# StarRocks/starrocks

Hardware: AMD Instinct MI355X
Metric: ssb_join_agg_rows_per_sec (higher is better)
Workload: dtype int64; 1 GPU; ssb_sf100_q21_star_groupby; rows_per_gpu=600000000, seed=42, parallelism=dp1-replicated-dims

## Files before the change

starrocks_amd/csrc/gpue.hip:

```cpp
#include <hip/hip_runtime.h>
#include <cstdio>
#include <cstring>
#include <cstdlib>
#include <thread>
#include "gpue.h"

static thread_local char g_err[512] = {0};

const char* gpue_last_error(void) { return g_err; }

#define HIP_CHECK(expr)                                                      \
    do {                                                                     \
        hipError_t _e = (expr);                                              \
        if (_e != hipSuccess) {                                              \
            snprintf(g_err, sizeof(g_err), "%s failed: %s (%s:%d)", #expr,   \
                     hipGetErrorString(_e), __FILE__, __LINE__);             \
            return GPUE_ERR_HIP;                                             \
        }                                                                    \
    } while (0)

#define ARG_CHECK(cond)                                                      \
    do {                                                                     \
        if (!(cond)) {                                                       \
            snprintf(g_err, sizeof(g_err), "bad argument: %s (%s:%d)",       \
// ... 3907 lines not shown
    uint32_t wqn = 0;
    const uint64_t n4 = n / 4;
    const int4* __restrict__ pk4 = (const int4*)pk;
    const int4* __restrict__ sk4 = (const int4*)sk;
    const int4* __restrict__ od4 = (const int4*)od;
    const int4* __restrict__ rv4 = (const int4*)rv;
    uint64_t stride = (uint64_t)gridDim.x * blockDim.x;
    auto ld4 = [&](const int4* p, uint64_t i) {
        const uint64_t* q = (const uint64_t*)(p + i);
        uint64_t lo = __builtin_nontemporal_load(q);
        uint64_t hi = __builtin_nontemporal_load(q + 1);
        int4 v;
        v.x = (int32_t)lo; v.y = (int32_t)(lo >> 32);
        v.z = (int32_t)hi; v.w = (int32_t)(hi >> 32);
        return v;
    };
    auto drain64 = [&]() {
        int4 e = wq[wid][wqn - 64 + lane];
        uint32_t brand1 = pfirst[e.x - 1];
        if (brand1) {
            uint32_t sidx = (uint32_t)(e.y - ssmin);
            if (sidx < ssint && ((sbits[sidx >> 5] >> (sidx & 31)) & 1u)) {
                uint32_t year1 = dfirst[e.z - dmin];
                atomicAdd(&g[(year1 - 1) * 1000 + (brand1 - 1)],
                          (unsigned long long)(int64_t)e.w);
            }
        }
        wqn -= 64;
    };
    auto quad = [&](int4 p4, int4 s4, int4 o4, int4 r4, bool inb) {
        #pragma unroll
        for (int j = 0; j < 4; j++) {
            uint32_t idx = (uint32_t)((&p4.x)[j] - psmin);
            bool in = inb & (idx < psint);
            uint32_t fidx = (in ? idx : 0u) & PF_MASK;
            bool maybe = in & (pf[fidx >> 5] >> (fidx & 31)) & 1u;
            uint64_t m = __ballot(maybe);
            if (m) {
                uint32_t rank = __popcll(m & ((1ull << lane) - 1));
                if (maybe)
                    wq[wid][wqn + rank] =
                        make_int4((&p4.x)[j], (&s4.x)[j], (&o4.x)[j], (&r4.x)[j]);
                wqn += __popcll(m);
                if (wqn >= 64) drain64();
            }
        }
    };
    uint64_t base = (uint64_t)blockIdx.x * blockDim.x + (uint64_t)wid * WAVE;
    uint64_t i = base + lane;
    for (; base + stride + WAVE <= n4; base += 2 * stride, i += 2 * stride) {
        int4 pa = ld4(pk4, i), sa = ld4(sk4, i), oa = ld4(od4, i), ra = ld4(rv4, i);
        uint64_t i2 = i + stride;
        int4 pb_ = ld4(pk4, i2), sb = ld4(sk4, i2), ob = ld4(od4, i2), rb = ld4(rv4, i2);
        quad(pa, sa, oa, ra, true);
        quad(pb_, sb, ob, rb, true);
    }
    for (; base < n4; base += stride, i += stride) {
        bool inb = i < n4;
        int4 z = make_int4(0, 0, 0, 0);
        int4 p4 = inb ? pk4[i] : z, s4 = inb ? sk4[i] : z;
        int4 o4 = inb ? od4[i] : z, r4 = inb ? rv4[i] : z;
        quad(p4, s4, o4, r4, inb);
    }
    if (wqn > 0 && lane < (int)wqn) {
        int4 e = wq[wid][lane];
        uint32_t brand1 = pfirst[e.x - 1];
        if (brand1) {
            uint32_t sidx = (uint32_t)(e.y - ssmin);
            if (sidx < ssint && ((sbits[sidx >> 5] >> (sidx & 31)) & 1u)) {
                uint32_t year1 = dfirst[e.z - dmin];
                atomicAdd(&g[(year1 - 1) * 1000 + (brand1 - 1)],
                          (unsigned long long)(int64_t)e.w);
            }
        }
    }
    uint64_t tid = (uint64_t)blockIdx.x * blockDim.x + threadIdx.x;
    for (uint64_t r = n4 * 4 + tid; r < n; r += stride) {
        uint32_t idx = (uint32_t)(pk[r] - psmin);
        if (idx >= psint) continue;
        uint32_t fidx = idx & PF_MASK;
        if (!((pf[fidx >> 5] >> (fidx & 31)) & 1u)) continue;
        uint32_t brand1 = pfirst[pk[r] - 1];
        if (!brand1) continue;
        uint32_t sidx = (uint32_t)(sk[r] - ssmin);
        if (sidx >= ssint || !((sbits[sidx >> 5] >> (sidx & 31)) & 1u)) continue;
        uint32_t year1 = dfirst[od[r] - dmin];
        atomicAdd(&g[(year1 - 1) * 1000 + (brand1 - 1)], (unsigned long long)(int64_t)rv[r]);
    }
    __syncthreads();
    for (int j = threadIdx.x; j < NG_Q21; j += blockDim.x)
        if (g[j] != 0) atomicAdd(&group_sums[j], g[j]);
}

__global__ __launch_bounds__(BLOCK_Q21) void
k_q21_star_agg_pfq2(const int32_t* __restrict__ pk, const int32_t* __restrict__ sk,
                   const int32_t* __restrict__ od, const int32_t* __restrict__ rv,
                   uint64_t n, const uint32_t* __restrict__ prefilter, int64_t psmin,
                   uint64_t psint, const uint16_t* __restrict__ pfirst,
                   const uint32_t* __restrict__ sbits, int64_t ssmin, uint64_t ssint,
                   const uint16_t* __restrict__ dfirst, int64_t dmin,
                   unsigned long long* __restrict__ group_sums) {
    __shared__ uint32_t pfa[1 << 13];
    __shared__ uint32_t pfb[1 << 13];
    __shared__ unsigned long long g[NG_Q21];
    __shared__ int4 wq[BLOCK_Q21 / WAVE][128];
    for (uint32_t w = threadIdx.x; w < (1u << 13); w += blockDim.x) {
        pfa[w] = prefilter[w];
        pfb[w] = prefilter[(1u << 13) + w];
    }
    for (int j = threadIdx.x; j < NG_Q21; j += blockDim.x) g[j] = 0;
    __syncthreads();
    const int wid = threadIdx.x / WAVE;
    const int lane = threadIdx.x & (WAVE - 1);
    uint32_t wqn = 0;
    const uint64_t n4 = n / 4;
    const int4* __restrict__ pk4 = (const int4*)pk;
    const int4* __restrict__ sk4 = (const int4*)sk;
    const int4* __restrict__ od4 = (const int4*)od;
    const int4* __restrict__ rv4 = (const int4*)rv;
    uint64_t stride = (uint64_t)gridDim.x * blockDim.x;
    auto ld4 = [&](const int4* p, uint64_t i) {
        const uint64_t* q = (const uint64_t*)(p + i);
        uint64_t lo = __builtin_nontemporal_load(q);
        uint64_t hi = __builtin_nontemporal_load(q + 1);
        int4 v;
        v.x = (int32_t)lo; v.y = (int32_t)(lo >> 32);
        v.z = (int32_t)hi; v.w = (int32_t)(hi >> 32);
        return v;
    };
    auto drain64 = [&]() {
        int4 e = wq[wid][wqn - 64 + lane];
        uint32_t brand1 = pfirst[e.x - 1];
        if (brand1) {
            uint32_t sidx = (uint32_t)(e.y - ssmin);
            if (sidx < ssint && ((sbits[sidx >> 5] >> (sidx & 31)) & 1u)) {
                uint32_t year1 = dfirst[e.z - dmin];
                atomicAdd(&g[(year1 - 1) * 1000 + (brand1 - 1)],
                          (unsigned long long)(int64_t)e.w);
            }
        }
        wqn -= 64;
    };
    auto quad = [&](int4 p4, int4 s4, int4 o4, int4 r4, bool inb) {
        #pragma unroll
        for (int j = 0; j < 4; j++) {
            uint32_t idx = (uint32_t)((&p4.x)[j] - psmin);
            bool in = inb & (idx < psint);
            uint32_t ia = (in ? idx : 0u) & ((1u << 18) - 1);
            uint32_t ib = ((in ? idx : 0u) * 2654435761u) >> 14;
            bool maybe = in & (pfa[ia >> 5] >> (ia & 31)) & (pfb[ib >> 5] >> (ib & 31)) & 1u;
            uint64_t m = __ballot(maybe);
            if (m) {
                uint32_t rank = __popcll(m & ((1ull << lane) - 1));
                if (maybe)
                    wq[wid][wqn + rank] =
                        make_int4((&p4.x)[j], (&s4.x)[j], (&o4.x)[j], (&r4.x)[j]);
                wqn += __popcll(m);
                if (wqn >= 64) drain64();
            }
        }
    };
    uint64_t base = (uint64_t)blockIdx.x * blockDim.x + (uint64_t)wid * WAVE;
    uint64_t i = base + lane;
    for (; base + stride + WAVE <= n4; base += 2 * stride, i += 2 * stride) {
        int4 pa = ld4(pk4, i), sa = ld4(sk4, i), oa = ld4(od4, i), ra = ld4(rv4, i);
        uint64_t i2 = i + stride;
        int4 pb_ = ld4(pk4, i2), sb = ld4(sk4, i2), ob = ld4(od4, i2), rb = ld4(rv4, i2);
        quad(pa, sa, oa, ra, true);
        quad(pb_, sb, ob, rb, true);
    }
    for (; base < n4; base += stride, i += stride) {
        bool inb = i < n4;
        int4 z = make_int4(0, 0, 0, 0);
        int4 p4 = inb ? pk4[i] : z, s4 = inb ? sk4[i] : z;
        int4 o4 = inb ? od4[i] : z, r4 = inb ? rv4[i] : z;
        quad(p4, s4, o4, r4, inb);
    }
    if (wqn > 0 && lane < (int)wqn) {
        int4 e = wq[wid][lane];
        uint32_t brand1 = pfirst[e.x - 1];
        if (brand1) {
            uint32_t sidx = (uint32_t)(e.y - ssmin);
            if (sidx < ssint && ((sbits[sidx >> 5] >> (sidx & 31)) & 1u)) {
                uint32_t year1 = dfirst[e.z - dmin];
                atomicAdd(&g[(year1 - 1) * 1000 + (brand1 - 1)],
                          (unsigned long long)(int64_t)e.w);
            }
        }
    }
    uint64_t tid = (uint64_t)blockIdx.x * blockDim.x + threadIdx.x;
    for (uint64_t r = n4 * 4 + tid; r < n; r += stride) {
        uint32_t idx = (uint32_t)(pk[r] - psmin);
        if (idx >= psint) continue;
        uint32_t ia = idx & ((1u << 18) - 1);
        uint32_t ib = (idx * 2654435761u) >> 14;
        if (!((pfa[ia >> 5] >> (ia & 31)) & (pfb[ib >> 5] >> (ib & 31)) & 1u)) continue;
        uint32_t brand1 = pfirst[pk[r] - 1];
        if (!brand1) continue;
        uint32_t sidx = (uint32_t)(sk[r] - ssmin);
        if (sidx >= ssint || !((sbits[sidx >> 5] >> (sidx & 31)) & 1u)) continue;
        uint32_t year1 = dfirst[od[r] - dmin];
        atomicAdd(&g[(year1 - 1) * 1000 + (brand1 - 1)], (unsigned long long)(int64_t)rv[r]);
    }
    __syncthreads();
    for (int j = threadIdx.x; j < NG_Q21; j += blockDim.x)
        if (g[j] != 0) atomicAdd(&group_sums[j], g[j]);
}


__global__ __launch_bounds__(BLOCK_Q21) void
k_q21_star_agg_pfq3(const int32_t* __restrict__ pk, const int32_t* __restrict__ sk,
                    const int32_t* __restrict__ od, const int32_t* __restrict__ rv,
                    uint64_t n, const uint32_t* __restrict__ prefilter, int64_t psmin,
                    uint64_t psint, const uint16_t* __restrict__ pfirst,
                    const uint32_t* __restrict__ sbits, int64_t ssmin, uint64_t ssint,
                    const uint16_t* __restrict__ dfirst, int64_t dmin,
                    unsigned long long* __restrict__ group_sums) {
    __shared__ uint32_t pfa[1 << 13];
    __shared__ uint32_t pfb[1 << 13];
    __shared__ unsigned long long g[NG_Q21];
    __shared__ int2 wq[BLOCK_Q21 / WAVE][128];
    for (uint32_t w = threadIdx.x; w < (1u << 13); w += blockDim.x) {
        pfa[w] = prefilter[w];
        pfb[w] = prefilter[(1u << 13) + w];
    }
    for (int j = threadIdx.x; j < NG_Q21; j += blockDim.x) g[j] = 0;
    __syncthreads();
    const int wid = threadIdx.x / WAVE;
    const int lane = threadIdx.x & (WAVE - 1);
    uint32_t wqn = 0;
    const uint64_t n4 = n / 4;
    const int4* __restrict__ pk4 = (const int4*)pk;
    uint64_t stride = (uint64_t)gridDim.x * blockDim.x;
    auto process = [&](int2 e) {
        uint32_t brand1 = pfirst[e.x - 1];
        if (!brand1) return;
        uint32_t r = (uint32_t)e.y;
        uint32_t sidx = (uint32_t)(sk[r] - ssmin);
        if (sidx >= ssint || !((sbits[sidx >> 5] >> (sidx & 31)) & 1u)) return;
        uint32_t year1 = dfirst[od[r] - dmin];
        atomicAdd(&g[(year1 - 1) * 1000 + (brand1 - 1)],
                  (unsigned long long)(int64_t)rv[r]);
    };
    auto push = [&](int32_t key, uint32_t row, bool inb) {
        uint32_t idx = (uint32_t)(key - psmin);
        bool in = inb & (idx < psint);
        uint32_t ia = (in ? idx : 0u) & ((1u << 18) - 1);
        uint32_t ib = ((in ? idx : 0u) * 2654435761u) >> 14;
        bool maybe = in & (pfa[ia >> 5] >> (ia & 31)) & (pfb[ib >> 5] >> (ib & 31)) & 1u;
        uint64_t m = __ballot(maybe);
        if (m) {
            uint32_t rank = __popcll(m & ((1ull << lane) - 1));
            if (maybe) wq[wid][wqn + rank] = make_int2(key, (int32_t)row);
            wqn += __popcll(m);
            if (wqn >= 64) {
                process(wq[wid][wqn - 64 + lane]);
                wqn -= 64;
            }
        }
    };
    auto ld4nt = [&](const int4* p, uint64_t i) {
        const uint64_t* q = (const uint64_t*)(p + i);
        uint64_t lo = __builtin_nontemporal_load(q);
        uint64_t hi = __builtin_nontemporal_load(q + 1);
        int4 v;
        v.x = (int32_t)lo; v.y = (int32_t)(lo >> 32);
        v.z = (int32_t)hi; v.w = (int32_t)(hi >> 32);
        return v;
    };
    uint64_t base = (uint64_t)blockIdx.x * blockDim.x + (uint64_t)wid * WAVE;
    uint64_t i = base + lane;
    for (; base + stride + WAVE <= n4; base += 2 * stride, i += 2 * stride) {
        int4 pa = ld4nt(pk4, i);
        uint64_t i2 = i + stride;
        int4 pb_ = ld4nt(pk4, i2);
        #pragma unroll
        for (int j = 0; j < 4; j++) push((&pa.x)[j], (uint32_t)(i * 4 + j), true);
        #pragma unroll
        for (int j = 0; j < 4; j++) push((&pb_.x)[j], (uint32_t)(i2 * 4 + j), true);
    }
    for (; base < n4; base += stride, i += stride) {
        bool inb = i < n4;
        int4 p4 = inb ? pk4[i] : make_int4(0, 0, 0, 0);
        #pragma unroll
        for (int j = 0; j < 4; j++) push((&p4.x)[j], (uint32_t)(i * 4 + j), inb);
    }
    if (wqn > 0 && lane < (int)wqn) process(wq[wid][lane]);
    uint64_t tid = (uint64_t)blockIdx.x * blockDim.x + threadIdx.x;
    for (uint64_t r = n4 * 4 + tid; r < n; r += stride) {
        uint32_t idx = (uint32_t)(pk[r] - psmin);
        if (idx >= psint) continue;
        uint32_t brand1 = pfirst[pk[r] - 1];
        if (!brand1) continue;
        uint32_t sidx = (uint32_t)(sk[r] - ssmin);
        if (sidx >= ssint || !((sbits[sidx >> 5] >> (sidx & 31)) & 1u)) continue;
        uint32_t year1 = dfirst[od[r] - dmin];
        atomicAdd(&g[(year1 - 1) * 1000 + (brand1 - 1)], (unsigned long long)(int64_t)rv[r]);
    }
    __syncthreads();
    for (int j = threadIdx.x; j < NG_Q21; j += blockDim.x)
        if (g[j] != 0) atomicAdd(&group_sums[j], g[j]);
}

__global__ void k_q21_pass_payload(const int32_t* __restrict__ pk, uint64_t n,
                                   const uint32_t* __restrict__ pbits, int64_t psmin,
                                   uint64_t psint, const uint16_t* __restrict__ pfirst,
                                   uint16_t* __restrict__ brand_out) {
    const uint64_t n4 = n / 4;
    const int4* __restrict__ pk4 = (const int4*)pk;
    uint64_t stride = (uint64_t)gridDim.x * blockDim.x;
    uint64_t i = (uint64_t)blockIdx.x * blockDim.x + threadIdx.x;
    for (; i + stride < n4; i += 2 * stride) {
        int4 pa = pk4[i];
        int4 pb_ = pk4[i + stride];
        ushort4 oa, ob;
        #pragma unroll
        for (int j = 0; j < 4; j++) {
            uint32_t idx = (uint32_t)((&pa.x)[j] - psmin);
            bool in = idx < psint;
            uint32_t cidx = in ? idx : 0u;
            bool pass = in & ((pbits[cidx >> 5] >> (cidx & 31)) & 1u);
            (&oa.x)[j] = pass ? pfirst[(&pa.x)[j] - 1] : (uint16_t)0;
        }
        #pragma unroll
        for (int j = 0; j < 4; j++) {
            uint32_t idx = (uint32_t)((&pb_.x)[j] - psmin);
            bool in = idx < psint;
            uint32_t cidx = in ? idx : 0u;
            bool pass = in & ((pbits[cidx >> 5] >> (cidx & 31)) & 1u);
            (&ob.x)[j] = pass ? pfirst[(&pb_.x)[j] - 1] : (uint16_t)0;
        }
        ((ushort4*)brand_out)[i] = oa;
        ((ushort4*)brand_out)[i + stride] = ob;
    }
    for (; i < n4; i += stride) {
        int4 p4 = pk4[i];
        ushort4 o;
        #pragma unroll
        for (int j = 0; j < 4; j++) {
            uint32_t idx = (uint32_t)((&p4.x)[j] - psmin);
            bool in = idx < psint;
            uint32_t cidx = in ? idx : 0u;
            bool pass = in & ((pbits[cidx >> 5] >> (cidx & 31)) & 1u);
            (&o.x)[j] = pass ? pfirst[(&p4.x)[j] - 1] : (uint16_t)0;
        }
        ((ushort4*)brand_out)[i] = o;
    }
    uint64_t tid = (uint64_t)blockIdx.x * blockDim.x + threadIdx.x;
    for (uint64_t r = n4 * 4 + tid; r < n; r += stride) {
        uint32_t idx = (uint32_t)(pk[r] - psmin);
        bool in = idx < psint;
        uint32_t cidx = in ? idx : 0u;
        bool pass = in & ((pbits[cidx >> 5] >> (cidx & 31)) & 1u);
        brand_out[r] = pass ? pfirst[pk[r] - 1] : (uint16_t)0;
    }
}

__global__ __launch_bounds__(BLOCK_Q21) void
k_q21_phase2(const uint16_t* __restrict__ brand, const int32_t* __restrict__ sk,
             const int32_t* __restrict__ od, const int32_t* __restrict__ rv, uint64_t n,
             const uint32_t* __restrict__ sbits, int64_t ssmin, uint64_t ssint,
             const uint16_t* __restrict__ dfirst, int64_t dmin,
             unsigned long long* __restrict__ group_sums) {
    __shared__ unsigned long long g[NG_Q21];
    for (int j = threadIdx.x; j < NG_Q21; j += blockDim.x) g[j] = 0;
    __syncthreads();
    const uint64_t n4 = n / 4;
    const ushort4* __restrict__ br4 = (const ushort4*)brand;
    const int4* __restrict__ sk4 = (const int4*)sk;
    const int4* __restrict__ od4 = (const int4*)od;
    const int4* __restrict__ rv4 = (const int4*)rv;
    uint64_t stride = (uint64_t)gridDim.x * blockDim.x;
    for (uint64_t i = (uint64_t)blockIdx.x * blockDim.x + threadIdx.x; i < n4; i += stride) {
        ushort4 b4 = br4[i];
        int4 s4 = sk4[i];
        int4 o4 = od4[i];
        int4 r4 = rv4[i];
        #pragma unroll
        for (int j = 0; j < 4; j++) {
            uint16_t brand1 = (&b4.x)[j];
            if (brand1 == 0) continue;
            uint32_t sidx = (uint32_t)((&s4.x)[j] - ssmin);
            if (sidx >= ssint || !((sbits[sidx >> 5] >> (sidx & 31)) & 1u)) continue;
            uint32_t year1 = dfirst[(&o4.x)[j] - dmin];
            atomicAdd(&g[(year1 - 1) * 1000 + (brand1 - 1)],
                      (unsigned long long)(int64_t)(&r4.x)[j]);
        }
    }
    uint64_t tid = (uint64_t)blockIdx.x * blockDim.x + threadIdx.x;
    for (uint64_t r = n4 * 4 + tid; r < n; r += stride) {
        uint16_t brand1 = brand[r];
        if (brand1 == 0) continue;
        uint32_t sidx = (uint32_t)(sk[r] - ssmin);
        if (sidx >= ssint || !((sbits[sidx >> 5] >> (sidx & 31)) & 1u)) continue;
        uint32_t year1 = dfirst[od[r] - dmin];
        atomicAdd(&g[(year1 - 1) * 1000 + (brand1 - 1)], (unsigned long long)(int64_t)rv[r]);
    }
    __syncthreads();
    for (int j = threadIdx.x; j < NG_Q21; j += blockDim.x)
        if (g[j] != 0) atomicAdd(&group_sums[j], g[j]);
}

extern "C" int gpue_q21_star_agg_pipe(gpue_session* s, gpue_join_table* parts,
                                      gpue_join_table* supps, gpue_join_table* dates,
                                      gpue_dbuf* pk, gpue_dbuf* sk, gpue_dbuf* od,
                                      gpue_dbuf* rv, uint64_t n, gpue_dbuf* brand_scratch,
                                      gpue_dbuf* group_sums, int n_chunks);
int gpue_q21_star_agg_pipe(gpue_session* s, gpue_join_table* parts, gpue_join_table* supps,
                           gpue_join_table* dates, gpue_dbuf* pk, gpue_dbuf* sk,
                           gpue_dbuf* od, gpue_dbuf* rv, uint64_t n,
                           gpue_dbuf* brand_scratch, gpue_dbuf* group_sums, int n_chunks) {
    ARG_CHECK(s && parts && supps && dates && pk && sk && od && rv && brand_scratch &&
              group_sums);
    ARG_CHECK(parts->first16 && parts->bitset && supps->bitset && dates->first16);
    ARG_CHECK(brand_scratch->bytes >= n * 2);
    ARG_CHECK(n_chunks >= 1 && n_chunks <= gpue_session::N_CHUNK_EVENTS);
    HIP_CHECK(hipMemsetAsync(group_sums->ptr, 0, NG_Q21 * sizeof(int64_t), s->stream));
    uint64_t per = (n + (uint64_t)n_chunks - 1) / (uint64_t)n_chunks;
    uint64_t chunk = (per + 3) & ~3ull;
    for (int c = 0; c < n_chunks; c++) {
        uint64_t lo = (uint64_t)c * chunk;
        if (lo >= n) break;
        uint64_t len = min(chunk, n - lo);
        hipLaunchKernelGGL(k_q21_pass_payload, dim3(grid_for(len)), dim3(BLOCK), 0,
                           s->stream2, (const int32_t*)pk->ptr + lo, len, parts->bitset,
                           parts->set_min, (uint64_t)(parts->set_max - parts->set_min + 1),
                           parts->first16, (uint16_t*)brand_scratch->ptr + lo);
        HIP_CHECK(hipEventRecord(s->chunk_ev[c], s->stream2));
        HIP_CHECK(hipStreamWaitEvent(s->stream, s->chunk_ev[c], 0));
        hipLaunchKernelGGL(k_q21_phase2, dim3(env_cap("GPUE_GRID_WIDE", 512)),
                           dim3(BLOCK_Q21), 0, s->stream,
                           (const uint16_t*)brand_scratch->ptr + lo,
                           (const int32_t*)sk->ptr + lo, (const int32_t*)od->ptr + lo,
                           (const int32_t*)rv->ptr + lo, len, supps->bitset,
                           supps->set_min, (uint64_t)(supps->set_max - supps->set_min + 1),
                           dates->first16, dates->min_key,
                           (unsigned long long*)group_sums->ptr);
    }
    HIP_CHECK(hipGetLastError());
    return GPUE_OK;
}

static bool q21_glob() {
    static int v = -1;
    if (v < 0) {
        const char* e = getenv("GPUE_Q21_GLOB");
        v = (e && atoi(e)) ? 1 : 0;
    }
    return v == 1;
}

static bool q21_pf() {
    static int v = -1;
    if (v < 0) {
        const char* e = getenv("GPUE_Q21_PF");
        v = (e && !atoi(e)) ? 0 : 1;
    }
    return v == 1;
}

extern "C" int gpue_q21_star_agg_async(gpue_session* s, gpue_join_table* parts,
                                       gpue_join_table* supps, gpue_join_table* dates,
                                       gpue_dbuf* pk, gpue_dbuf* sk, gpue_dbuf* od,
                                       gpue_dbuf* rv, uint64_t n, gpue_dbuf* group_sums);
int gpue_q21_star_agg_async(gpue_session* s, gpue_join_table* parts, gpue_join_table* supps,
                            gpue_join_table* dates, gpue_dbuf* pk, gpue_dbuf* sk,
                            gpue_dbuf* od, gpue_dbuf* rv, uint64_t n, gpue_dbuf* group_sums) {
    ARG_CHECK(s && parts && supps && dates && pk && sk && od && rv && group_sums);
    ARG_CHECK(group_sums->bytes >= NG_Q21 * sizeof(int64_t));
    ARG_CHECK(parts->min_key == 1 && supps->min_key == 1);
    ARG_CHECK(parts->first16 && supps->first16 && dates->first16);
    HIP_CHECK(hipMemsetAsync(group_sums->ptr, 0, NG_Q21 * sizeof(int64_t), s->stream));
    if (q21_pf() && parts->prefilter) {
        const char* e = getenv("GPUE_Q21_PF");
        int mode = e ? atoi(e) : 7;
        const char* nt = getenv("GPUE_Q21_PF_NT");
        bool use_nt = !nt || atoi(nt);
        int def_grid = mode == 2 ? 512 : 256;
        int tpb = env_cap("GPUE_Q21_PF_TPB", BLOCK_Q21);
        auto launch = [&](auto kern, int grid) {
            hipLaunchKernelGGL(kern, dim3(env_cap("GPUE_GRID_PF", grid)),
                               dim3(tpb), 0, s->stream, (const int32_t*)pk->ptr,
                               (const int32_t*)sk->ptr, (const int32_t*)od->ptr,
                               (const int32_t*)rv->ptr, n, parts->prefilter, parts->set_min,
                               (uint64_t)(parts->set_max - parts->set_min + 1),
                               parts->first16, supps->bitset, supps->set_min,
                               (uint64_t)(supps->set_max - supps->set_min + 1),
                               dates->first16, dates->min_key,
                               (unsigned long long*)group_sums->ptr);
        };
        if (mode == 7) {
            hipLaunchKernelGGL(k_q21_star_agg_pfq3, dim3(env_cap("GPUE_GRID_PF", def_grid)),
                               dim3(tpb), 0, s->stream, (const int32_t*)pk->ptr,
                               (const int32_t*)sk->ptr, (const int32_t*)od->ptr,
                               (const int32_t*)rv->ptr, n, parts->prefilter2,
                               parts->set_min,
                               (uint64_t)(parts->set_max - parts->set_min + 1),
                               parts->first16, supps->bitset, supps->set_min,
                               (uint64_t)(supps->set_max - supps->set_min + 1),
                               dates->first16, dates->min_key,
                               (unsigned long long*)group_sums->ptr);
        }
        else if (mode == 6) {
            hipLaunchKernelGGL(k_q21_star_agg_pfq2, dim3(env_cap("GPUE_GRID_PF", def_grid)),
                               dim3(tpb), 0, s->stream, (const int32_t*)pk->ptr,
                               (const int32_t*)sk->ptr, (const int32_t*)od->ptr,
                               (const int32_t*)rv->ptr, n, parts->prefilter2,
                               parts->set_min,
                               (uint64_t)(parts->set_max - parts->set_min + 1),
                               parts->first16, supps->bitset, supps->set_min,
                               (uint64_t)(supps->set_max - supps->set_min + 1),
                               dates->first16, dates->min_key,
                               (unsigned long long*)group_sums->ptr);
        }
        else if (mode == 4) launch(k_q21_star_agg_pfq, def_grid);
        else if (mode == 2 && use_nt) launch(k_q21_star_agg_pf<false, true>, def_grid);
        else if (mode == 2) launch(k_q21_star_agg_pf<false, false>, def_grid);
        else if (use_nt) launch(k_q21_star_agg_pf<true, true>, def_grid);
        else launch(k_q21_star_agg_pf<true, false>, def_grid);
        HIP_CHECK(hipGetLastError());
        return GPUE_OK;
    }
    if (q21_glob()) {
        hipLaunchKernelGGL(k_q21_star_agg_glob, dim3(grid_stream(n)), dim3(BLOCK), 0,
                           s->stream, (const int32_t*)pk->ptr, (const int32_t*)sk->ptr,
                           (const int32_t*)od->ptr, (const int32_t*)rv->ptr, n,
                           parts->bitset, parts->set_min,
                           (uint64_t)(parts->set_max - parts->set_min + 1), parts->first16,
                           supps->bitset, supps->set_min,
                           (uint64_t)(supps->set_max - supps->set_min + 1), dates->first16,
                           dates->min_key, (unsigned long long*)group_sums->ptr);
    } else
    hipLaunchKernelGGL(k_q21_star_agg, dim3(env_cap("GPUE_GRID_WIDE", 512)), dim3(BLOCK_Q21), 0, s->stream,
                       (const int32_t*)pk->ptr, (const int32_t*)sk->ptr,
                       (const int32_t*)od->ptr, (const int32_t*)rv->ptr, n,
                       parts->bitset, parts->set_min,
                       (uint64_t)(parts->set_max - parts->set_min + 1), parts->first16,
                       supps->bitset, supps->set_min,
                       (uint64_t)(supps->set_max - supps->set_min + 1), dates->first16,
                       dates->min_key, (unsigned long long*)group_sums->ptr);
    HIP_CHECK(hipGetLastError());
    return GPUE_OK;
}

int gpue_q21_star_agg(gpue_session* s, gpue_join_table* parts, gpue_join_table* supps,
                      gpue_join_table* dates, gpue_dbuf* pk, gpue_dbuf* sk, gpue_dbuf* od,
                      gpue_dbuf* rv, uint64_t n, int64_t* group_sums_out) {
    ARG_CHECK(s && parts && supps && dates && pk && sk && od && rv && group_sums_out);
    ARG_CHECK(pk->bytes >= n * 4 && sk->bytes >= n * 4 && od->bytes >= n * 4 && rv->bytes >= n * 4);
    ARG_CHECK(parts->min_key == 1 && supps->min_key == 1);
    ARG_CHECK(parts->first16 && supps->first16 && dates->first16);
    unsigned long long* d_g = nullptr;
    HIP_CHECK(hipMalloc(&d_g, NG_Q21 * sizeof(unsigned long long)));
    gpue_dbuf tmp{s, d_g, NG_Q21 * sizeof(unsigned long long), false};
    int rc = gpue_q21_star_agg_async(s, parts, supps, dates, pk, sk, od, rv, n, &tmp);
    if (rc != GPUE_OK) {
        (void)hipFree(d_g);
        return rc;
    }
    HIP_CHECK(hipMemcpyAsync(group_sums_out, d_g, NG_Q21 * sizeof(int64_t),
                             hipMemcpyDeviceToHost, s->stream));
    HIP_CHECK(hipStreamSynchronize(s->stream));
    (void)hipFree(d_g);
    return GPUE_OK;
}

static constexpr int NG_Q43 = 800;

template <bool PF>
__global__ __launch_bounds__(BLOCK_Q21) void
k_q43_star_agg(const int32_t* __restrict__ ck, const int32_t* __restrict__ sk,
               const int32_t* __restrict__ pk, const int32_t* __restrict__ od,
               const int32_t* __restrict__ rv, const int32_t* __restrict__ sc,
               uint64_t n, const uint32_t* __restrict__ prefilter,
               const uint32_t* __restrict__ cbits, int64_t csmin, uint64_t csint,
               const uint32_t* __restrict__ sbits, int64_t ssmin, uint64_t ssint,
               const uint16_t* __restrict__ sfirst,
               const uint32_t* __restrict__ pbits, int64_t psmin, uint64_t psint,
               const uint16_t* __restrict__ pfirst,
               const uint16_t* __restrict__ dfirst, int64_t dmin,
               unsigned long long* __restrict__ group_sums) {
    __shared__ unsigned long long g[NG_Q43];
    __shared__ uint32_t pf[PF ? PF_WORDS : 1];
    if (PF)
        for (uint32_t w = threadIdx.x; w < PF_WORDS; w += blockDim.x) pf[w] = prefilter[w];
    for (int j = threadIdx.x; j < NG_Q43; j += blockDim.x) g[j] = 0;
    __syncthreads();
    const uint64_t n4 = n / 4;
    const int4* __restrict__ ck4 = (const int4*)ck;
    const int4* __restrict__ sk4 = (const int4*)sk;
    const int4* __restrict__ pk4 = (const int4*)pk;
    const int4* __restrict__ od4 = (const int4*)od;
    uint64_t stride = (uint64_t)gridDim.x * blockDim.x;
    auto quad_mask = [&](int4 p4) -> uint32_t {
        uint32_t m = 0;
        #pragma unroll
        for (int j = 0; j < 4; j++) {
            uint32_t idx = (uint32_t)((&p4.x)[j] - psmin);
            uint32_t cidx = idx < psint ? idx : 0u;
            if (PF) {
                uint32_t fidx = cidx & PF_MASK;
                bool maybe = (idx < psint) & (pf[fidx >> 5] >> (fidx & 31)) & 1u;
                if (maybe) m |= ((pbits[cidx >> 5] >> (cidx & 31)) & 1u) << j;
            } else {
                m |= ((idx < psint) & (pbits[cidx >> 5] >> (cidx & 31)) & 1u) << j;
            }
        }
        return m;
    };
    auto quad_rest = [&](uint32_t m, uint64_t q, int4 c4, int4 s4, int4 p4, int4 o4) {
        #pragma unroll
        for (int j = 0; j < 4; j++) {
            if (!((m >> j) & 1u)) continue;
            uint32_t sidx = (uint32_t)((&s4.x)[j] - ssmin);
            if (sidx >= ssint || !((sbits[sidx >> 5] >> (sidx & 31)) & 1u)) continue;
            uint32_t cidx = (uint32_t)((&c4.x)[j] - csmin);
            if (cidx >= csint || !((cbits[cidx >> 5] >> (cidx & 31)) & 1u)) continue;
            uint32_t dpay = dfirst[(&o4.x)[j] - dmin];
            if (dpay == 0) continue;
            uint32_t ppay = pfirst[(&p4.x)[j] - 1];
            uint32_t spay = sfirst[(&s4.x)[j] - 1];
            uint64_t r = q * 4 + j;
            atomicAdd(&g[(dpay - 1) * 400 + (spay - 1) * 40 + (ppay - 1)],
                      (unsigned long long)((int64_t)rv[r] - sc[r]));
        }
    };
    uint64_t i = (uint64_t)blockIdx.x * blockDim.x + threadIdx.x;
    for (; i + stride < n4; i += 2 * stride) {
        int4 pa = pk4[i];
        uint64_t i2 = i + stride;
        int4 pb_ = pk4[i2];
        uint32_t ma = quad_mask(pa), mb = quad_mask(pb_);
        if (ma) quad_rest(ma, i, ck4[i], sk4[i], pa, od4[i]);
        if (mb) quad_rest(mb, i2, ck4[i2], sk4[i2], pb_, od4[i2]);
    }
    for (; i < n4; i += stride) {
        int4 p4 = pk4[i];
        uint32_t m = quad_mask(p4);
        if (m) quad_rest(m, i, ck4[i], sk4[i], p4, od4[i]);
    }
    uint64_t tid = (uint64_t)blockIdx.x * blockDim.x + threadIdx.x;
    for (uint64_t r = n4 * 4 + tid; r < n; r += stride) {
        uint32_t pidx = (uint32_t)(pk[r] - psmin);
        if (pidx >= psint || !((pbits[pidx >> 5] >> (pidx & 31)) & 1u)) continue;
        uint32_t sidx = (uint32_t)(sk[r] - ssmin);
        if (sidx >= ssint || !((sbits[sidx >> 5] >> (sidx & 31)) & 1u)) continue;
        uint32_t cidx = (uint32_t)(ck[r] - csmin);
        if (cidx >= csint || !((cbits[cidx >> 5] >> (cidx & 31)) & 1u)) continue;
        uint32_t dpay = dfirst[od[r] - dmin];
        if (dpay == 0) continue;
        uint32_t ppay = pfirst[pk[r] - 1];
        uint32_t spay = sfirst[sk[r] - 1];
        atomicAdd(&g[(dpay - 1) * 400 + (spay - 1) * 40 + (ppay - 1)],
                  (unsigned long long)((int64_t)rv[r] - sc[r]));
    }
    __syncthreads();
    for (int j = threadIdx.x; j < NG_Q43; j += blockDim.x)
        if (g[j] != 0) atomicAdd(&group_sums[j], g[j]);
}

__global__ __launch_bounds__(BLOCK_Q21) void
k_q43_star_agg_pfq(const int32_t* __restrict__ ck, const int32_t* __restrict__ sk,
                   const int32_t* __restrict__ pk, const int32_t* __restrict__ od,
                   const int32_t* __restrict__ rv, const int32_t* __restrict__ sc,
                   uint64_t n, const uint32_t* __restrict__ prefilter,
                   const uint32_t* __restrict__ cbits, int64_t csmin, uint64_t csint,
                   const uint32_t* __restrict__ sbits, int64_t ssmin, uint64_t ssint,
                   const uint16_t* __restrict__ sfirst,
                   const uint32_t* __restrict__ pbits, int64_t psmin, uint64_t psint,
                   const uint16_t* __restrict__ pfirst,
                   const uint16_t* __restrict__ dfirst, int64_t dmin,
                   unsigned long long* __restrict__ group_sums) {
    __shared__ uint32_t pf[PF_WORDS];
    __shared__ unsigned long long g[NG_Q43];
    __shared__ int2 wq[BLOCK_Q21 / WAVE][128];
    for (uint32_t w = threadIdx.x; w < PF_WORDS; w += blockDim.x) pf[w] = prefilter[w];
    for (int j = threadIdx.x; j < NG_Q43; j += blockDim.x) g[j] = 0;
    __syncthreads();
    const int wid = threadIdx.x / WAVE;
    const int lane = threadIdx.x & (WAVE - 1);
    uint32_t wqn = 0;
    const uint64_t n4 = n / 4;
    const int4* __restrict__ pk4 = (const int4*)pk;
    uint64_t stride = (uint64_t)gridDim.x * blockDim.x;
    auto process = [&](int2 e) {
        uint32_t idx = (uint32_t)(e.x - psmin);
        if (!((pbits[idx >> 5] >> (idx & 31)) & 1u)) return;
        uint32_t r = (uint32_t)e.y;
        int32_t skv = sk[r];
        uint32_t sidx = (uint32_t)(skv - ssmin);
        if (sidx >= ssint || !((sbits[sidx >> 5] >> (sidx & 31)) & 1u)) return;
        uint32_t cidx = (uint32_t)(ck[r] - csmin);
        if (cidx >= csint || !((cbits[cidx >> 5] >> (cidx & 31)) & 1u)) return;
        uint32_t dpay = dfirst[od[r] - dmin];
        if (dpay == 0) return;
        uint32_t ppay = pfirst[e.x - 1];
        uint32_t spay = sfirst[skv - 1];
        atomicAdd(&g[(dpay - 1) * 400 + (spay - 1) * 40 + (ppay - 1)],
                  (unsigned long long)((int64_t)rv[r] - sc[r]));
    };
    auto push = [&](int32_t key, uint32_t row, bool inb) {
        uint32_t idx = (uint32_t)(key - psmin);
        bool in = inb & (idx < psint);
        uint32_t fidx = (in ? idx : 0u) & PF_MASK;
        bool maybe = in & (pf[fidx >> 5] >> (fidx & 31)) & 1u;
        uint64_t m = __ballot(maybe);
        if (m) {
            uint32_t rank = __popcll(m & ((1ull << lane) - 1));
            if (maybe) wq[wid][wqn + rank] = make_int2(key, (int32_t)row);
            wqn += __popcll(m);
            if (wqn >= 64) {
                process(wq[wid][wqn - 64 + lane]);
                wqn -= 64;
            }
        }
    };
    uint64_t base = (uint64_t)blockIdx.x * blockDim.x + (uint64_t)wid * WAVE;
    uint64_t i = base + lane;
    for (; base + stride + WAVE <= n4; base += 2 * stride, i += 2 * stride) {
        int4 pa = pk4[i];
        uint64_t i2 = i + stride;
        int4 pb_ = pk4[i2];
        #pragma unroll
        for (int j = 0; j < 4; j++) push((&pa.x)[j], (uint32_t)(i * 4 + j), true);
        #pragma unroll
        for (int j = 0; j < 4; j++) push((&pb_.x)[j], (uint32_t)(i2 * 4 + j), true);
    }
    for (; base < n4; base += stride, i += stride) {
        bool inb = i < n4;
        int4 p4 = inb ? pk4[i] : make_int4(0, 0, 0, 0);
        #pragma unroll
        for (int j = 0; j < 4; j++) push((&p4.x)[j], (uint32_t)(i * 4 + j), inb);
    }
    if (wqn > 0 && lane < (int)wqn) process(wq[wid][lane]);
    uint64_t tid = (uint64_t)blockIdx.x * blockDim.x + threadIdx.x;
    for (uint64_t r = n4 * 4 + tid; r < n; r += stride) {
        uint32_t pidx = (uint32_t)(pk[r] - psmin);
        if (pidx >= psint || !((pbits[pidx >> 5] >> (pidx & 31)) & 1u)) continue;
        uint32_t sidx = (uint32_t)(sk[r] - ssmin);
        if (sidx >= ssint || !((sbits[sidx >> 5] >> (sidx & 31)) & 1u)) continue;
        uint32_t cidx = (uint32_t)(ck[r] - csmin);
        if (cidx >= csint || !((cbits[cidx >> 5] >> (cidx & 31)) & 1u)) continue;
        uint32_t dpay = dfirst[od[r] - dmin];
        if (dpay == 0) continue;
        uint32_t ppay = pfirst[pk[r] - 1];
        uint32_t spay = sfirst[sk[r] - 1];
        atomicAdd(&g[(dpay - 1) * 400 + (spay - 1) * 40 + (ppay - 1)],
                  (unsigned long long)((int64_t)rv[r] - sc[r]));
    }
    __syncthreads();
    for (int j = threadIdx.x; j < NG_Q43; j += blockDim.x)
        if (g[j] != 0) atomicAdd(&group_sums[j], g[j]);
}

__global__ __launch_bounds__(BLOCK_Q21) void
k_q43_star_agg_pfq2(const int32_t* __restrict__ ck, const int32_t* __restrict__ sk,
                   const int32_t* __restrict__ pk, const int32_t* __restrict__ od,
                   const int32_t* __restrict__ rv, const int32_t* __restrict__ sc,
                   uint64_t n, const uint32_t* __restrict__ prefilter,
                   const uint32_t* __restrict__ cbits, int64_t csmin, uint64_t csint,
                   const uint32_t* __restrict__ sbits, int64_t ssmin, uint64_t ssint,
                   const uint16_t* __restrict__ sfirst,
                   const uint32_t* __restrict__ pbits, int64_t psmin, uint64_t psint,
                   const uint16_t* __restrict__ pfirst,
                   const uint16_t* __restrict__ dfirst, int64_t dmin,
                   unsigned long long* __restrict__ group_sums) {
    __shared__ uint32_t pfa[PF_WORDS];
    __shared__ uint32_t pfb[PF_WORDS];
    __shared__ unsigned long long g[NG_Q43];
    __shared__ int2 wq[BLOCK_Q21 / WAVE][128];
    for (uint32_t w = threadIdx.x; w < PF_WORDS; w += blockDim.x) {
        pfa[w] = prefilter[w];
        pfb[w] = prefilter[PF_WORDS + w];
    }
    for (int j = threadIdx.x; j < NG_Q43; j += blockDim.x) g[j] = 0;
    __syncthreads();
    const int wid = threadIdx.x / WAVE;
    const int lane = threadIdx.x & (WAVE - 1);
    uint32_t wqn = 0;
    const uint64_t n4 = n / 4;
    const int4* __restrict__ pk4 = (const int4*)pk;
    uint64_t stride = (uint64_t)gridDim.x * blockDim.x;
    auto process = [&](int2 e) {
        uint32_t idx = (uint32_t)(e.x - psmin);
        if (!((pbits[idx >> 5] >> (idx & 31)) & 1u)) return;
        uint32_t r = (uint32_t)e.y;
        int32_t skv = sk[r];
        uint32_t sidx = (uint32_t)(skv - ssmin);
        if (sidx >= ssint || !((sbits[sidx >> 5] >> (sidx & 31)) & 1u)) return;
        uint32_t cidx = (uint32_t)(ck[r] - csmin);
        if (cidx >= csint || !((cbits[cidx >> 5] >> (cidx & 31)) & 1u)) return;
        uint32_t dpay = dfirst[od[r] - dmin];
        if (dpay == 0) return;
        uint32_t ppay = pfirst[e.x - 1];
// ... 4320 lines not shown
```

Before: 537.5 billion rows/s.

## Add multi-stage wave-queue Q21 kernel with software prefetch of part keys

Adds a new Q21 star-join aggregation kernel and makes it the default mode. It chains wave-local compaction queues: a two-hash bloom prefilter on the part key, then the part brand lookup, then the supplier bitset check, and only after that the date and revenue gathers. It also software-pipelines the nontemporal part-key loads so the next iteration's keys are fetched while the current ones are processed. The goal is to keep lanes busy and coalesce the dependent random gathers, at the cost of extra LDS use and queue bookkeeping that may reduce occupancy.

```diff
diff --git a/starrocks_amd/csrc/gpue.hip b/starrocks_amd/csrc/gpue.hip
--- a/starrocks_amd/csrc/gpue.hip
+++ b/starrocks_amd/csrc/gpue.hip
@@ -4233,6 +4233,196 @@
         if (g[j] != 0) atomicAdd(&group_sums[j], g[j]);
 }
 
+template <bool PREFETCH, int B>
+__global__ __launch_bounds__(BLOCK_Q21) void
+k_q21_star_agg_pfq4(const int32_t* __restrict__ pk, const int32_t* __restrict__ sk,
+                    const int32_t* __restrict__ od, const int32_t* __restrict__ rv,
+                    uint64_t n, const uint32_t* __restrict__ prefilter, int64_t psmin,
+                    uint64_t psint, const uint16_t* __restrict__ pfirst,
+                    const uint32_t* __restrict__ sbits, int64_t ssmin, uint64_t ssint,
+                    const uint16_t* __restrict__ dfirst, int64_t dmin,
+                    unsigned long long* __restrict__ group_sums) {
+    constexpr int B3 = B > 0 ? B : 1;
+    constexpr int QS = B > 0 ? 126 + 64 * B3 : 1;
+    __shared__ uint32_t pfa[1 << 13];
+    __shared__ uint32_t pfb[1 << 13];
+    __shared__ unsigned long long g[NG_Q21];
+    __shared__ int2 q1[BLOCK_Q21 / WAVE][128];
+    __shared__ uint32_t qrow[BLOCK_Q21 / WAVE][QS];
+    __shared__ uint16_t qbr[BLOCK_Q21 / WAVE][QS];
+    for (uint32_t w = threadIdx.x; w < (1u << 13); w += blockDim.x) {
+        pfa[w] = prefilter[w];
+        pfb[w] = prefilter[(1u << 13) + w];
+    }
+    for (int j = threadIdx.x; j < NG_Q21; j += blockDim.x) g[j] = 0;
+    __syncthreads();
+    const int wid = threadIdx.x / WAVE;
+    const uint32_t lane = threadIdx.x & (WAVE - 1);
+    const uint64_t below = (1ull << lane) - 1;
+    uint32_t n1 = 0, n2 = 0, n3 = 0;
+    const uint64_t n4 = n / 4;
+    const int4* __restrict__ pk4 = (const int4*)pk;
+    uint64_t stride = (uint64_t)gridDim.x * blockDim.x;
+    auto drain3 = [&](uint32_t cnt) {
+        uint32_t r[B3], b[B3], y[B3];
+        int32_t o[B3], v[B3];
+        bool act[B3];
+        #pragma unroll
+        for (int k = 0; k < B3; k++) {
+            act[k] = k * 64 + lane < cnt;
+            uint32_t slot = QS - 1 - (n3 - cnt + k * 64 + lane);
+            r[k] = act[k] ? qrow[wid][slot] : 0u;
+            b[k] = act[k] ? qbr[wid][slot] : 0u;
+        }
+        n3 -= cnt;
+        #pragma unroll
+        for (int k = 0; k < B3; k++)
+            if (act[k]) {
+                o[k] = od[r[k]];
+                v[k] = rv[r[k]];
+            }
+        #pragma unroll
+        for (int k = 0; k < B3; k++)
+            if (act[k]) y[k] = dfirst[o[k] - dmin];
+        #pragma unroll
+        for (int k = 0; k < B3; k++)
+            if (act[k])
+                atomicAdd(&g[(y[k] - 1) * 1000 + (b[k] - 1)],
+                          (unsigned long long)(int64_t)v[k]);
+    };
+    auto drain2 = [&](uint32_t cnt) {
+        bool act = lane < cnt;
+        uint32_t r = act ? qrow[wid][n2 - cnt + lane] : 0u;
+        uint32_t b = act ? qbr[wid][n2 - cnt + lane] : 0u;
+        n2 -= cnt;
+        bool pass = false;
+        if (act) {
+            uint32_t sidx = (uint32_t)(sk[r] - ssmin);
+            pass = sidx < ssint && ((sbits[sidx >> 5] >> (sidx & 31)) & 1u);
+        }
+        uint64_t m = __ballot(pass);
+        if (m) {
+            if (pass) {
+                uint32_t slot = QS - 1 - (n3 + __popcll(m & below));
+                qrow[wid][slot] = r;
+                qbr[wid][slot] = (uint16_t)b;
+            }
+            n3 += __popcll(m);
+            if (n3 >= 64 * B3) drain3(64 * B3);
+        }
+    };
+    auto drain1 = [&](uint32_t cnt) {
+        bool act = lane < cnt;
+        int2 e = act ? q1[wid][n1 - cnt + lane] : make_int2(1, 0);
+        n1 -= cnt;
+        uint32_t brand1 = act ? pfirst[e.x - 1] : 0u;
+        if constexpr (B == 0) {
+            if (!brand1) return;
+            uint32_t r = (uint32_t)e.y;
+            uint32_t sidx = (uint32_t)(sk[r] - ssmin);
+            if (sidx >= ssint || !((sbits[sidx >> 5] >> (sidx & 31)) & 1u)) return;
+            uint32_t year1 = dfirst[od[r] - dmin];
+            atomicAdd(&g[(year1 - 1) * 1000 + (brand1 - 1)],
+                      (unsigned long long)(int64_t)rv[r]);
+        } else {
+            uint64_t m = __ballot(brand1 != 0);
+            if (m) {
+                if (brand1) {
+                    uint32_t slot = n2 + __popcll(m & below);
+                    qrow[wid][slot] = (uint32_t)e.y;
+                    qbr[wid][slot] = (uint16_t)brand1;
+                }
+                n2 += __popcll(m);
+                if (n2 >= 64) drain2(64);
+            }
+        }
+    };
+    auto push = [&](int32_t key, uint32_t row, bool inb) {
+        uint32_t idx = (uint32_t)(key - psmin);
+        bool in = inb & (idx < psint);
+        uint32_t ia = (in ? idx : 0u) & ((1u << 18) - 1);
+        uint32_t ib = ((in ? idx : 0u) * 2654435761u) >> 14;
+        bool maybe = in & (pfa[ia >> 5] >> (ia & 31)) & (pfb[ib >> 5] >> (ib & 31)) & 1u;
+        uint64_t m = __ballot(maybe);
+        if (m) {
+            if (maybe) q1[wid][n1 + __popcll(m & below)] = make_int2(key, (int32_t)row);
+            n1 += __popcll(m);
+            if (n1 >= 64) drain1(64);
+        }
+    };
+    auto ld4nt = [&](const int4* p, uint64_t i) {
+        const uint64_t* q = (const uint64_t*)(p + i);
+        uint64_t lo = __builtin_nontemporal_load(q);
+        uint64_t hi = __builtin_nontemporal_load(q + 1);
+        int4 v;
+        v.x = (int32_t)lo; v.y = (int32_t)(lo >> 32);
+        v.z = (int32_t)hi; v.w = (int32_t)(hi >> 32);
+        return v;
+    };
+    uint64_t base = (uint64_t)blockIdx.x * blockDim.x + (uint64_t)wid * WAVE;
+    uint64_t i = base + lane;
+    if constexpr (PREFETCH) {
+        bool more = base + stride + WAVE <= n4;
+        int4 pa = make_int4(0, 0, 0, 0), pb_ = pa;
+        if (more) {
+            pa = ld4nt(pk4, i);
+            pb_ = ld4nt(pk4, i + stride);
+        }
+        while (more) {
+            const uint64_t ci = i, ci2 = i + stride;
+            base += 2 * stride;
+            i += 2 * stride;
+            more = base + stride + WAVE <= n4;
+            int4 na = pa, nb = pb_;
+            if (more) {
+                na = ld4nt(pk4, i);
+                nb = ld4nt(pk4, i + stride);
+            }
+            #pragma unroll
+            for (int j = 0; j < 4; j++) push((&pa.x)[j], (uint32_t)(ci * 4 + j), true);
+            #pragma unroll
+            for (int j = 0; j < 4; j++) push((&pb_.x)[j], (uint32_t)(ci2 * 4 + j), true);
+            pa = na;
+            pb_ = nb;
+        }
+    } else {
+        for (; base + stride + WAVE <= n4; base += 2 * stride, i += 2 * stride) {
+            int4 pa = ld4nt(pk4, i);
+            uint64_t i2 = i + stride;
+            int4 pb_ = ld4nt(pk4, i2);
+            #pragma unroll
+            for (int j = 0; j < 4; j++) push((&pa.x)[j], (uint32_t)(i * 4 + j), true);
+            #pragma unroll
+            for (int j = 0; j < 4; j++) push((&pb_.x)[j], (uint32_t)(i2 * 4 + j), true);
+        }
+    }
+    for (; base < n4; base += stride, i += stride) {
+        bool inb = i < n4;
+        int4 p4 = inb ? pk4[i] : make_int4(0, 0, 0, 0);
+        #pragma unroll
+        for (int j = 0; j < 4; j++) push((&p4.x)[j], (uint32_t)(i * 4 + j), inb);
+    }
+    if (n1 > 0) drain1(n1);
+    if constexpr (B > 0) {
+        if (n2 > 0) drain2(n2);
+        if (n3 > 0) drain3(n3);
+    }
+    uint64_t tid = (uint64_t)blockIdx.x * blockDim.x + threadIdx.x;
+    for (uint64_t r = n4 * 4 + tid; r < n; r += stride) {
+        uint32_t idx = (uint32_t)(pk[r] - psmin);
+        if (idx >= psint) continue;
+        uint32_t brand1 = pfirst[pk[r] - 1];
+        if (!brand1) continue;
+        uint32_t sidx = (uint32_t)(sk[r] - ssmin);
+        if (sidx >= ssint || !((sbits[sidx >> 5] >> (sidx & 31)) & 1u)) continue;
+        uint32_t year1 = dfirst[od[r] - dmin];
+        atomicAdd(&g[(year1 - 1) * 1000 + (brand1 - 1)], (unsigned long long)(int64_t)rv[r]);
+    }
+    __syncthreads();
+    for (int j = threadIdx.x; j < NG_Q21; j += blockDim.x)
+        if (g[j] != 0) atomicAdd(&group_sums[j], g[j]);
+}
+
 __global__ void k_q21_pass_payload(const int32_t* __restrict__ pk, uint64_t n,
                                    const uint32_t* __restrict__ pbits, int64_t psmin,
                                    uint64_t psint, const uint16_t* __restrict__ pfirst,
@@ -4404,7 +4594,7 @@
     HIP_CHECK(hipMemsetAsync(group_sums->ptr, 0, NG_Q21 * sizeof(int64_t), s->stream));
     if (q21_pf() && parts->prefilter) {
         const char* e = getenv("GPUE_Q21_PF");
-        int mode = e ? atoi(e) : 7;
+        int mode = e ? atoi(e) : 8;
         const char* nt = getenv("GPUE_Q21_PF_NT");
         bool use_nt = !nt || atoi(nt);
         int def_grid = mode == 2 ? 512 : 256;
@@ -4420,7 +4610,28 @@
                                dates->first16, dates->min_key,
                                (unsigned long long*)group_sums->ptr);
         };
-        if (mode == 7) {
+        ARG_CHECK((mode != 7 && mode != 8) || n <= UINT32_MAX);
+        if (mode == 8) {
+            auto launch8 = [&](auto kern) {
+                hipLaunchKernelGGL(kern, dim3(env_cap("GPUE_GRID_PF", def_grid)),
+                                   dim3(tpb), 0, s->stream, (const int32_t*)pk->ptr,
+                                   (const int32_t*)sk->ptr, (const int32_t*)od->ptr,
+                                   (const int32_t*)rv->ptr, n, parts->prefilter2,
+                                   parts->set_min,
+                                   (uint64_t)(parts->set_max - parts->set_min + 1),
+                                   parts->first16, supps->bitset, supps->set_min,
+                                   (uint64_t)(supps->set_max - supps->set_min + 1),
+                                   dates->first16, dates->min_key,
+                                   (unsigned long long*)group_sums->ptr);
+            };
+            int var = (int)env_cap("GPUE_Q21_PF8_VAR", 11);
+            ARG_CHECK(var == 10 || var == 1 || var == 11 || var == 12);
+            if (var == 10) launch8(k_q21_star_agg_pfq4<true, 0>);
+            else if (var == 1) launch8(k_q21_star_agg_pfq4<false, 1>);
+            else if (var == 11) launch8(k_q21_star_agg_pfq4<true, 1>);
+            else launch8(k_q21_star_agg_pfq4<true, 2>);
+        }
+        else if (mode == 7) {
             hipLaunchKernelGGL(k_q21_star_agg_pfq3, dim3(env_cap("GPUE_GRID_PF", def_grid)),
                                dim3(tpb), 0, s->stream, (const int32_t*)pk->ptr,
                                (const int32_t*)sk->ptr, (const int32_t*)od->ptr,
```

Result: faster. 582.8 billion rows/s, median of 6 (+8.4%).
